# arancormonk/dsd-neo

Measured on AMD Instinct MI355X. Metric: I/Q Msamples/s end-to-end (demod->FEC->MBE) per GPU; % HBM roofline, higher is better.
Workload: dtype f32

## Files before the change

### dsd-neo_amd/csrc/ddn_rx.hip

```cpp

#include <hip/hip_runtime.h>
#include <cstdio>
#include <cstdlib>
#include <mutex>
#include <stdint.h>

#include "ddn_device.h"
#include "ddn_p25h_dev.h"
#include "ddn_slicer_dev.h"
#include "ddn_tables_p25.h"

using ddn_sl::two_max_insert;
using ddn_sl::two_min_insert;

#define DDN_RXW_RAW (1 << 30)
namespace {
constexpr int TS = 64;
constexpr int SS = 128;
constexpr int MS = 1024;
constexpr int NT = DDN_P25_FILTER_TAPS;
constexpr int QCAP = 10;
constexpr uint32_t kSyncBits = 0xFB30A0u;

__constant__ uint32_t c_taps[NT];
// ... 1715 lines not shown
        s.max = (float)(s.max_sum / (double)MS);
        s.center = (s.max + s.min) / 2.0f;
        s.maxref = s.max * 0.80f;
        s.minref = s.min * 0.80f;
        s.sidx = (s.sidx >= SS - 1) ? 0 : s.sidx + 1;
        fl = 1 | (neg ? 4 : 0);
        q_max = s.max;
        q_min = s.min;
        if (--s.lock_left <= 0) {
            if (HM && s.hphase != 0) {
                hpost = true;
            } else {
                frame_end();
            }
        }
    };
    auto commit_hunt = [&](float sym, int done_snap, int& fl) {
        L.lb[s.lidx][ln] = sym;
        s.level_count = s.level_count < 24 ? s.level_count + 1 : 24;
        float u0, u1, u2, u3;
        window_push(sym, false, u0, u1, u2, u3, done_snap);
        s.lidx = (s.lidx == 23) ? 0 : s.lidx + 1;
        s.sidx = (s.sidx >= SS - 1) ? 0 : s.sidx + 1;
        const uint32_t bit = sym > 0.0f ? 1u : 0u;
        s.hist_bits = ((s.hist_bits << 1) | bit) & 0xFFFFFFu;
        s.hist_count = s.hist_count < 24 ? s.hist_count + 1 : 24;
        if (s.hist_count >= 8) {
            s.maxref = s.max;
            s.minref = s.min;
            int pol = 0;
            if (s.hist_count >= 24) {
                pol = (s.hist_bits == kSyncBits) ? 1 : ((s.hist_bits == (~kSyncBits & 0xFFFFFFu)) ? 2 : 0);
            }
            if (pol) {
                const float big = 3.4028234663852886e38f;
                float a0 = big, a1 = big, a2 = big, a3 = big, a4 = big;
                float b0 = -big, b1 = -big, b2 = -big, b3 = -big, b4 = -big;
                const int lc = s.level_count;
#pragma unroll 4
                for (int k = 0; k < 24; k++) {
                    const float x = L.lb[k][ln];
                    float v = k < lc ? x : big, t;
                    float w = k < lc ? x : -big;
                    t = fminf(a0, v); v = fmaxf(a0, v); a0 = t;
                    t = fminf(a1, v); v = fmaxf(a1, v); a1 = t;
                    t = fminf(a2, v); v = fmaxf(a2, v); a2 = t;
                    t = fminf(a3, v); v = fmaxf(a3, v); a3 = t;
                    a4 = fminf(a4, v);
                    t = fmaxf(b0, w); w = fminf(b0, w); b0 = t;
                    t = fmaxf(b1, w); w = fminf(b1, w); b1 = t;
                    t = fmaxf(b2, w); w = fminf(b2, w); b2 = t;
                    t = fmaxf(b3, w); w = fminf(b3, w); b3 = t;
                    b4 = fmaxf(b4, w);
                }
                if (lc >= 13) {
                    s.lmin = (a2 + a3 + a4) / 3.0f;
                    s.lmax = (b4 + b3 + b2) / 3.0f;
                } else {
                    s.lmin = (a0 + a1 + a2) / 3.0f;
                    s.lmax = (b2 + b1 + b0) / 3.0f;
                }
                s.max = (s.max + s.lmax) / 2;
                s.min = (s.min + s.lmin) / 2;
                s.lastsync = pol;
                if (use_flt && !s.filter_on) {
                    s.filter_on = 1;
                    s.filt_start = abs0 + t0 + sp;
                    cold_until = sp + (NT - 1);
                }
                if (s.scount >= 24) {
                    float sp_ = 0.0f, sn_ = 0.0f;
                    int np = 0, nn = 0;
                    int idx = s.shead;
#pragma unroll 4
                    for (int k = 0; k < 24; k++) {
                        idx = idx == 0 ? 23 : idx - 1;
                        const float v = L.sh[idx][ln];
                        const bool pos = v > 0.0f;
                        sp_ += pos ? v : 0.0f;
                        sn_ += pos ? 0.0f : v;
                        np += pos ? 1 : 0;
                        nn += pos ? 0 : 1;
                    }
                    if (np != 0 && nn != 0) {
                        const float mp = sp_ / (float)np, mn = sn_ / (float)nn;
                        if (!(fabsf(mp - mn) < 1.0f)) {
                            s.max = mp;
                            s.min = mn;
                            s.center = (s.max + s.min) / 2.0f;
                            s.umid = s.center + (s.max - s.center) * 0.625f;
                            s.lmid = s.center + (s.min - s.center) * 0.625f;
                            s.maxref = s.max * 0.80f;
                            s.minref = s.min * 0.80f;
                            s.fill_max = s.max;
                            s.fill_min = s.min;
                            fill_max_d = (double)s.max;
                            fill_min_d = (double)s.min;
                            s.since_fill = 0;
                            s.max_sum = (double)s.max * (double)MS;
                            s.min_sum = (double)s.min * (double)MS;
                        }
                    }
                }
                s.have_sync = 1;
                s.lock_left = lock_cfg[ch];
                if (HM) {
                    s.lock_left = 33;
                    s.hphase = 1;
                    s.hn = 33;
                }
                fl = 2 | (pol == 2 ? 4 : 0);
                if (s.lock_left <= 0) {
                    s.have_sync = 0;
                    s.lidx = 0;
                    s.level_count = 0;
                    s.hist_count = 0;
                    s.hist_bits = 0;
                    s.lmin = s.min;
                    s.lmax = s.max;
                    s.hunt_pos = 0;
                }
            }
        }
        if (!(fl & 2)) {
            hunt_advance();
        }
    };
    auto emit = [&](float sym, int fl, float q_max, float q_min) {
    if (fl & 1) {
        hist_push(sym, q_max, q_min, fl);
    }
    if (offload && tk <= QTW) {
        qv = make_float4(sym, q_max, q_min, __int_as_float(fl | ((o - o_tile) << 8)));
    } else if ((size_t)o < max_sym) {
        int dibit, relb = 0, l0 = 0, l1 = 0;
        if (fl & 1) {
            const float center = (q_max + q_min) / 2.0f;
            const ddn_sl::Thr th = {center, ((q_max - center) * 5.0f / 8.0f) + center,
                                    ((q_min - center) * 5.0f / 8.0f) + center, q_max, q_min};
            ddn_sl::slice_soft(sym, th, (fl >> 2) & 1, dibit, relb, l0, l1);
        } else {
            dibit = sym > 0.0f ? 1 : 3;
        }
        store_record(rp + (size_t)o * 10, fp + o, sym, dibit, relb, l0, l1, fl);
    }
        o++;
    };

    long long dbg_busy = 0, dbg_wait = 0, dbg_cyc[3] = {0, 0, 0}, dbg_prev = 0, dbg_sec[8] = {0, 0, 0, 0, 0, 0, 0, 0}, dbg_st = 0;
#define DBG_SEC(k) do { if (DDN_RX_CYCLES && (cfg.dbg & 8192)) { const long long n_ = (long long)clock64(); dbg_sec[k] += n_ - dbg_st; dbg_st = n_; } } while (0)
    int dbg_n[3] = {0, 0, 0}, dbg_kind = -1;
    long long dbg_blk[8] = {0, 0, 0, 0, 0, 0, 0, 0}, dbg_bt = 0;
#define DBG_BLK(k) do { if (DDN_RX_CYCLES && (cfg.dbg & 8192)) { const long long n_ = (long long)clock64(); dbg_blk[k] += n_ - dbg_bt; dbg_bt = n_; } } while (0)
    long long dbg_run[8] = {0, 0, 0, 0, 0, 0, 0, 0};
    long long dbg_ent[8] = {0, 0, 0, 0, 0, 0, 0, 0};
    if (HM && loader) {
        const int n_tiles = (int)((n + TW - 1) / TW);
        int job[NRW];
        for (int h = 0; h < NRW; h++) {
            job[h] = 0;
        }
        float idle_spin = 0.0f;
        auto jobs_left = [&]() {
            bool any = false;
            for (int h = 0; h < NRW; h++) {
                any = any || job[h] <= n_tiles;
            }
            return any;
        };
        while (jobs_left()) {
            bool served = false;
#pragma unroll
            for (int h = 0; h < NRW; h++) {
                const int j = job[h];
                const int tdw = __hip_atomic_load(&H.tile_done[h], __ATOMIC_RELAXED, __HIP_MEMORY_SCOPE_WORKGROUP);
                if (j > n_tiles || (tdw & (DDN_RXW_RAW - 1)) < j) {
                    continue;
                }
                __builtin_amdgcn_fence(__ATOMIC_ACQUIRE, "workgroup");
                const long long w0 = (DDN_RX_CYCLES && (cfg.dbg & 8192)) ? (long long)clock64() : 0;
                if (j < n_tiles) {
                    long long c0 = w0;
                    StageRegs sg;
                    if (j + 1 < n_tiles) {
                        stage_half_load((long)(j + 1) * TW, h, sg, (tdw & DDN_RXW_RAW) != 0);
                    }
                    if (DDN_RX_CYCLES && (cfg.dbg & 8192)) {
                        const long long c1 = (long long)clock64();
                        dbg_cyc[0] += c1 - c0;
                        c0 = c1;
                    }
                    if (offload && j > 0 && !(cfg.dbg & 512)) {
                        drain_half((j - 1) & 1, h);
                    }
                    if (DDN_RX_CYCLES && (cfg.dbg & 8192)) {
                        const long long c1 = (long long)clock64();
                        dbg_cyc[1] += c1 - c0;
                        c0 = c1;
                    }
                    if (fuse_mf) {
                        if (j + 1 < n_tiles) {
                            stage_half_store(j + 1, h, sg);
                        }
                        __builtin_amdgcn_fence(__ATOMIC_RELEASE, "workgroup");
                        if (lane == 0) {
                            __hip_atomic_store(&H.staged[h], j + 2, __ATOMIC_RELAXED, __HIP_MEMORY_SCOPE_WORKGROUP);
                        }
                        if (DDN_RX_CYCLES && (cfg.dbg & 8192)) {
                            const long long c1 = (long long)clock64();
                            dbg_cyc[0] += c1 - c0;
                            c0 = c1;
                        }
                    }
                    if (j >= 1 && !(cfg.dbg & 256)) {
                        compute_sfx_half(j & 1, j & 1, h);
                    }
                    if (DDN_RX_CYCLES && (cfg.dbg & 8192)) {
                        const long long c1 = (long long)clock64();
                        dbg_cyc[2] += c1 - c0;
                        c0 = c1;
                    }
                    if (!fuse_mf && j + 1 < n_tiles) {
                        stage_half_store(j + 1, h, sg);
                    }
                    if (DDN_RX_CYCLES && (cfg.dbg & 8192)) {
                        dbg_cyc[0] += (long long)clock64() - c0;
                    }
                    __builtin_amdgcn_fence(__ATOMIC_RELEASE, "workgroup");
                    if (lane == 0) {
                        __hip_atomic_store(&H.ready[h], j + 2, __ATOMIC_RELAXED, __HIP_MEMORY_SCOPE_WORKGROUP);
                    }
                } else if (offload && n_tiles > 0) {
                    drain_half((n_tiles - 1) & 1, h);
                }
                if (DDN_RX_CYCLES && (cfg.dbg & 8192)) {
                    dbg_busy += (long long)clock64() - w0;
                }
                job[h] = j + 1;
                served = true;
            }
            if (!served) {
                const long long w0 = (DDN_RX_CYCLES && (cfg.dbg & 8192)) ? (long long)clock64() : 0;
                helper_idle(idle_spin, (cfg.dbg & 8388608) != 0, 1);
                if (DDN_RX_CYCLES && (cfg.dbg & 8192)) {
                    dbg_wait += (long long)clock64() - w0;
                }
            }
        }
        it = n_tiles;
    } else
    for (t0 = 0; t0 < n; t0 += TW, it++) {
        const long long dbg_t0 = (DDN_RX_CYCLES && (cfg.dbg & 8192)) ? (long long)clock64() : 0;
        const int tn = (int)((n - t0) < TW ? (n - t0) : TW);
        const bool more = (t0 + TW) < n;
        long long dbg_spin = 0;
        if (HM) {
            const long long w0 = (DDN_RX_CYCLES && (cfg.dbg & 8192)) ? (long long)clock64() : 0;
            while (__hip_atomic_load(&H.ready[rw], __ATOMIC_RELAXED, __HIP_MEMORY_SCOPE_WORKGROUP) <= it
                   || (fuse_mf && __hip_atomic_load(&H.fready[rw], __ATOMIC_RELAXED, __HIP_MEMORY_SCOPE_WORKGROUP) <= it)) {
                __builtin_amdgcn_s_sleep(1);
            }
            __builtin_amdgcn_fence(__ATOMIC_ACQUIRE, "workgroup");
            if (DDN_RX_CYCLES && (cfg.dbg & 8192)) {
                dbg_spin = (long long)clock64() - w0;
            }
        }
        if (loader || winprep) {
            if (loader) {
                if (more) {
                    stage(t0 + TW, (it + 1) % 3);
                }
                if (offload && it > 0 && !(cfg.dbg & 512)) {
                    drain((it - 1) & 1);
                }
            }
            if (winprep) {
                if (it >= 1 && !(cfg.dbg & 256)) {
                    compute_sfx(it & 1, it & 1);
                }
            }
        } else {
            const int base = TW + (it % 3) * TW;
            auto rd = [&](const float* row, int j) { return row[base + j]; };
            auto cold_limit = [&]() {
                if (!s.filter_on) {
                    return -2147483647;
                }
                const long long d = (long long)(NT - 1) - (abs0 + t0 - s.filt_start);
                return d <= -2147483647LL ? -2147483647 : (d > 1000000LL ? 1000000 : (int)d);
            };
            cold_until = cold_limit();
            if (it >= 1) {
                pp1 = pc1, pp2 = pc2, pp3 = pc3, pp4 = pc4;
                npp = npc;
                sbuf_sel = (it - 1) & 1;
            }
            pc1 = inf, pc2 = inf, pc3 = -inf, pc4 = -inf;
            npc = 0;
            tk = 0;
            itq = it & 1;
            o_tile = o;
            if (live && offload) {
                L.qo[it & 1][ln] = o;
            }
            int guard = 0;
            bool gblocked = false;
            bool respin = false;
            int blk_o = -1;
            while (true) {
                const long long dbg_p0 = (DDN_RX_CYCLES && (cfg.dbg & 8192)) ? (long long)clock64() : 0;
                long long dbg_p1 = 0;
                if (HM && __any(hwait)) {
                    if (hwait
                        && __hip_atomic_load(&H.rsp_seq[ln], __ATOMIC_RELAXED, __HIP_MEMORY_SCOPE_WORKGROUP) == hseq) {
                        __builtin_amdgcn_fence(__ATOMIC_ACQUIRE, "workgroup", "local");
                        const int ext = H.rsp_ext[ln];
                        hwait = false;
                        if ((cfg.dbg & 65536) && !(cfg.dbg & (67108864 | 134217728))) {
                            s.dbg_wait += (long long)clock64();
                        }
#if DDN_RX_CYCLES
                        if (cfg.dbg & 67108864) {
                            s.dbg_wait += (long long)((int)clock64() - H.rsp_t[ln]);
                        }
                        if (cfg.dbg & 134217728) {
                            s.dbg_wait += (long long)H.rsp_pick[ln];
                        }
#endif
                        if (ext > 0) {
                            s.lock_left = ext;
                            s.hn = ext;
                            s.hphase = H.rsp_more[ln] ? 2 : 0;
                        } else {
                            s.hphase = 0;
                            frame_end();
                        }
                    }
                    if (__any(hwait) && (LPR > 4) != ((cfg.dbg & 262144) != 0)) {
                        __builtin_amdgcn_s_sleep(1);
                        continue;
                    }
                }
                const bool alive = live & !hwait;
                bool hunt_wait = false;
                if (bulk_ok) {
                    const int jt = s.jitter;
                    const int i0n = (jt > 0 && jt <= (whole - 1) / 2) ? -1 : ((jt > (whole - 1) / 2 && jt < whole) ? 1 : 0);
                    const bool be = alive & (s.have_sync == 0) & (s.in_symbol == 0) & (s.need_reset == 0) & (sp >= cold_until)
                                    & (s.hunt_pos + 20 < 1800) & (blk_o != o) & ((size_t)(o + 20) < max_sym);
                    const bool fitsn = sp + whole - i0n <= tn;
                    hunt_wait = be & !fitsn & more;
                    unsigned long long bm = __ballot(be & fitsn);
                    if constexpr (LPR == 2 || LPR == 4) {
                    if (__builtin_expect(bm != 0, 0)) {
                        const long long bt0 = (DDN_RX_CYCLES && (cfg.dbg & 8192)) ? (long long)clock64() : 0;
                        constexpr int OW = 64 / LPR;
                        constexpr int CAP = OW < 17 ? OW - 1 : 16;
                        constexpr unsigned long long GM = OW == 32 ? 0xFFFFFFFFull : 0xFFFFull;
                        const int g = lane / OW, l = lane % OW;
                        const bool gact = ((bm >> g) & 1ull) != 0;
                        const int cln = rw * LPR + g;
                        const int sp0 = __shfl(sp, g);
                        const float cen_o = __shfl(s.center, g), ls_o = __shfl(s.lastsample, g);
                        const float* pr = (__shfl(s.filter_on, g) ? &L.flt[cln][0] : &L.raw[cln][0]) + base;
                        int m = 0, mypk = 0;
                        if ((bm & (bm - 1)) == 0 || (cfg.dbg & 4096)) {
                            unsigned long long b2 = bm;
                            while (b2) {
                                const int ow = __ffsll((long long)b2) - 1;
                                b2 &= b2 - 1;
                                const int sp0s = __builtin_amdgcn_readlane(sp, ow), c0s = __builtin_amdgcn_readlane(s.hist_count, ow);
                                const float cen_s = __shfl(s.center, ow), ls_s = __shfl(s.lastsample, ow);
                                float hl = __shfl(s.maxref * 1.25f, ow), ll = __shfl(s.minref * 1.25f, ow);
                                const float hl_n = __shfl(s.max * 1.25f, ow), ll_n = __shfl(s.min * 1.25f, ow);
                                const float* prs = (__builtin_amdgcn_readlane(s.filter_on, ow) ? &L.flt[rw * LPR + ow][0] : &L.raw[rw * LPR + ow][0]) + base;
                                int q = sp0s, sm = 0, jit = __builtin_amdgcn_readlane(s.jitter, ow);
                                int lim = c0s < 8 ? 8 - c0s : CAP;
                                for (int ph = 0; ph < 2; ph++) {
                                    unsigned long long cm[3];
                                    q = __builtin_amdgcn_readfirstlane(q);
                                    sm = __builtin_amdgcn_readfirstlane(sm);
                                    jit = __builtin_amdgcn_readfirstlane(jit);
#pragma unroll
                                    for (int r = 0; r < 3; r++) {
                                        cm[r] = 0ull;
                                        if (q + 64 * r < tn) {
                                            const int a = q + lane + 64 * r;
                                            bool hit = false;
                                            if (a < tn) {
                                                const float x = prs[a];
                                                const float xp = (a == sp0s) ? ls_s : prs[a - 1];
                                                hit = (x > cen_s) ? (!(x > hl) && xp < cen_s) : (!(x < ll) && xp > cen_s);
                                            }
                                            cm[r] = __ballot(hit);
                                        }
                                    }
                                    bool full = false;
                                    auto uni64 = [](unsigned long long v) {
                                        const uint32_t lo = (uint32_t)__builtin_amdgcn_readfirstlane((int)(uint32_t)v);
                                        const uint32_t hi = (uint32_t)__builtin_amdgcn_readfirstlane((int)(uint32_t)(v >> 32));
                                        return ((unsigned long long)hi << 32) | lo;
                                    };
                                    cm[0] = uni64(cm[0]);
                                    cm[1] = uni64(cm[1]);
                                    cm[2] = uni64(cm[2]);
                                    while (sm < lim) {
                                        const int c = (int)((i0tab >> (2 * (jit + 1))) & 3u), i0 = c - 1;
                                        const int cnt = whole - i0;
                                        if (q + cnt > tn) {
                                            full = true;
                                            break;
                                        }
                                        asm("s_mov_b32 m0, %2\n\tv_writelane_b32 %0, %1, m0" : "+v"(mypk) : "s"((q + 256) | (c << 10) | ((jit + 1) << 12)), "s"(ow * OW + sm) : "m0");
                                        const int k0 = i0 < 0 ? 1 : 0;
                                        const uint32_t wv = (uint32_t)(cm[0] >> k0) & ((1u << (cnt - k0)) - 1u);
                                        jit = wv ? i0 + k0 + (__ffs((int)wv) - 1) : -1;
                                        cm[0] = (cm[0] >> cnt) | (cm[1] << (64 - cnt));
                                        cm[1] = (cm[1] >> cnt) | (cm[2] << (64 - cnt));
                                        cm[2] >>= cnt;
                                        q += cnt;
                                        sm++;
                                    }
                                    if (full || lim >= CAP) {
                                        break;
                                    }
                                    lim = CAP;
                                    hl = hl_n;
                                    ll = ll_n;
                                }
                                asm("s_mov_b32 m0, %2\n\tv_writelane_b32 %0, %1, m0" : "+v"(mypk) : "s"((q + 256) | ((jit + 1) << 12)), "s"(ow * OW + sm) : "m0");
                                m = g == ow ? sm : m;
                            }
                        } else {
                            int jit = __shfl(s.jitter, g), q = sp0;
                            float hl = __shfl(s.maxref * 1.25f, g), ll = __shfl(s.minref * 1.25f, g);
                            int lim = __shfl(s.hist_count, g);
                            lim = lim < 8 ? 8 - lim : CAP;
                            bool gdone = !gact;
                            for (int ph = 0; ph < 2; ph++) {
                                unsigned long long cm0 = 0ull, cm1 = 0ull, cm2 = 0ull;
                                constexpr int PW = 64 / OW;
#pragma unroll 1
                                for (int wd = 0; wd < 3; wd++) {
                                    unsigned long long word = 0ull;
#pragma unroll
                                    for (int r = 0; r < PW; r++) {
                                        const int a = q + l + OW * (wd * PW + r);
                                        bool hit = false;
                                        if (!gdone && a < tn) {
                                            const float x = pr[a];
                                            const float xp = (a == sp0) ? ls_o : pr[a - 1];
                                            hit = (x > cen_o) ? (!(x > hl) && xp < cen_o) : (!(x < ll) && xp > cen_o);
                                        }
                                        word |= ((__ballot(hit) >> (g * OW)) & GM) << (OW * r);
                                    }
                                    cm0 = wd == 0 ? word : cm0;
                                    cm1 = wd == 1 ? word : cm1;
                                    cm2 = wd == 2 ? word : cm2;
                                }
                                bool full = false;
                                while (true) {
                                    const bool go = !gdone && !full && m < lim;
                                    if (!__any(go)) {
                                        break;
                                    }
                                    if (go) {
                                        const int c = (int)((i0tab >> (2 * (jit + 1))) & 3u), i0 = c - 1;
                                        const int cnt = whole - i0;
                                        if (q + cnt > tn) {
                                            full = true;
                                        } else {
                                            if (l == m) {
                                                mypk = (q + 256) | (c << 10) | ((jit + 1) << 12);
                                            }
                                            const int k0 = i0 < 0 ? 1 : 0;
                                            const uint32_t wv = (uint32_t)(cm0 >> k0) & ((1u << (cnt - k0)) - 1u);
                                            jit = wv ? i0 + k0 + (__ffs((int)wv) - 1) : -1;
                                            cm0 = (cm0 >> cnt) | (cm1 << (64 - cnt));
                                            cm1 = (cm1 >> cnt) | (cm2 << (64 - cnt));
                                            cm2 >>= cnt;
                                            q += cnt;
                                            m++;
                                        }
                                    }
                                }
                                if (ph == 1) {
                                    break;
                                }
                                const float hl_n = __shfl(s.max * 1.25f, g), ll_n = __shfl(s.min * 1.25f, g);
                                if (!gdone) {
                                    if (full || lim >= CAP) {
                                        gdone = true;
                                    } else {
                                        lim = CAP;
                                        hl = hl_n;
                                        ll = ll_n;
                                    }
                                }
                                if (!__any(!gdone)) {
                                    break;
                                }
                            }
                            if (l == m) {
                                mypk = (q + 256) | ((jit + 1) << 12);
                            }
                        }
                        const int myq = (mypk & 1023) - 256, myi0 = ((mypk >> 10) & 3) - 1, myjin = ((mypk >> 12) & 15) - 1;
                        const int c0 = __shfl(s.hist_count, g);
                        const uint32_t h0 = (uint32_t)__shfl((int)s.hist_bits, g);
                        float sym = 0.0f;
                        if (gact && l < m) {
                            const float* pw = pr + myq + ((whole - 1) / 2 - 2 - myi0);
                            float acc = 0.0f;
#pragma unroll
                            for (int w = 0; w < 5; w++) {
                                acc += __builtin_amdgcn_fmed3f(pw[w], -inf, inf);
                            }
                            sym = acc / 5.0f;
                        }
                        const uint32_t sw = (uint32_t)((__ballot(gact && l < m && sym > 0.0f) >> (g * OW)) & GM);
                        const int lj = l < 31 ? l : 31;
                        const uint32_t hj = ((h0 << (lj + 1)) | __brev(sw << (31 - lj))) & 0xFFFFFFu;
                        const bool syn = gact && l < m && (c0 + l + 1 >= 24) && (hj == kSyncBits || hj == (~kSyncBits & 0xFFFFFFu));
                        const uint32_t smg = (uint32_t)((__ballot(syn) >> (g * OW)) & GM);
                        if (smg) {
                            m = __ffs((int)smg) - 1;
                        }
                        const int o_o = __shfl(o, g);
                        const int sh_o = __shfl(s.shead, g), li_o = __shfl(s.lidx, g), si_o = __shfl(s.sidx, g);
                        if (gact && l < m) {
                            int k = sh_o + l;
                            L.sh[k >= 24 ? k - 24 : k][cln] = sym;
                            k = li_o + l;
                            L.lb[k >= 24 ? k - 24 : k][cln] = sym;
                            L.sb[(si_o + l) & (SS - 1)][cln] = sym;
                            const size_t oo = (size_t)(o_o + l);
                            if (oo < max_sym) {
                                const size_t cho = (size_t)(ch0 + cln);
                                store_record(rec + (cho * max_sym + oo) * 10, flags + cho * max_sym + oo, sym, sym > 0.0f ? 1 : 3, 0, 0, 0, 0);
                            }
                        }
                        float a1 = (gact && l < m) ? sym : inf, a2 = inf, b1 = (gact && l < m) ? sym : -inf, b2 = -inf;
#define DDN_ROW_STEP(ctl)                                                                                                                   \
    do {                                                                                                                                    \
        const float o1 = __int_as_float(__builtin_amdgcn_update_dpp(0, __float_as_int(a1), ctl, 0xF, 0xF, true));                           \
        const float o2 = __int_as_float(__builtin_amdgcn_update_dpp(0, __float_as_int(a2), ctl, 0xF, 0xF, true));                           \
        const float p1 = __int_as_float(__builtin_amdgcn_update_dpp(0, __float_as_int(b1), ctl, 0xF, 0xF, true));                           \
        const float p2 = __int_as_float(__builtin_amdgcn_update_dpp(0, __float_as_int(b2), ctl, 0xF, 0xF, true));                           \
        two_min_insert(o1, a1, a2);                                                                                                         \
        two_min_insert(o2, a1, a2);                                                                                                         \
        two_max_insert(p1, b1, b2);                                                                                                         \
        two_max_insert(p2, b1, b2);                                                                                                         \
    } while (0)
                        DDN_ROW_STEP(0xB1);
                        DDN_ROW_STEP(0x4E);
                        DDN_ROW_STEP(0x124);
                        DDN_ROW_STEP(0x128);
#undef DDN_ROW_STEP
                        const int orow = (lane < LPR ? lane : 0) * OW;
                        const int m_own = __shfl(m, orow);
                        const int src1 = orow + (m_own > 0 ? m_own - 1 : 0);
                        const int qf = __shfl(myq, orow + m_own), jf = __shfl(myjin, orow + m_own);
                        const int il = __shfl(myi0, src1);
                        const uint32_t hf = (uint32_t)__shfl((int)hj, src1);
                        a1 = __shfl(a1, orow), a2 = __shfl(a2, orow), b1 = __shfl(b1, orow), b2 = __shfl(b2, orow);
                        if (lane < LPR && (be & fitsn)) {
                            if (m_own == 0) {
                                blk_o = o;
                            } else {
                                const float* prow = (s.filter_on ? &L.flt[ln][0] : &L.raw[ln][0]) + base;
                                const float lsf = prow[qf - 1];
                                two_min_insert(a1, pc1, pc2);
                                two_min_insert(a2, pc1, pc2);
                                two_max_insert(b1, pc3, pc4);
                                two_max_insert(b2, pc3, pc4);
                                npc += m_own;
                                wabs = fmaxf(wabs, fmaxf(fabsf(a1), fabsf(b1)));
                                s.shead = (s.shead + m_own) % 24;
                                s.scount = s.scount + m_own < 24 ? s.scount + m_own : 24;
                                s.lidx = (s.lidx + m_own) % 24;
                                s.level_count = s.level_count + m_own < 24 ? s.level_count + m_own : 24;
                                s.sidx = (s.sidx + m_own) & (SS - 1);
                                s.hist_bits = hf;
                                s.hist_count = s.hist_count + m_own < 24 ? s.hist_count + m_own : 24;
                                if (s.hist_count >= 8) {
                                    s.maxref = s.max;
                                    s.minref = s.min;
                                }
                                s.hunt_pos += m_own;
                                s.span = whole;
                                s.centre = (whole - 1) / 2;
                                s.i = il;
                                s.sum = 0.0f;
                                s.count = 0;
                                s.in_symbol = 0;
                                s.jitter = jf;
                                s.lastsample = lsf;
                                sp = qf;
                                o += m_own;
                            }
                        }
                        if (DDN_RX_CYCLES && (cfg.dbg & 8192)) {
                            const long long now = (long long)clock64();
                            dbg_sec[6] += now - bt0;
                            dbg_sec[7]++;
                            dbg_prev += now - bt0;
                        }
                        continue;
                    }
                    } else
                    if (__builtin_expect(bm != 0, 0)) {
                        const long long bt0 = (DDN_RX_CYCLES && (cfg.dbg & 8192)) ? (long long)clock64() : 0;
                        while (bm) {
                            const int ow = __ffsll((long long)bm) - 1;
                            bm &= bm - 1;
                            if (DDN_RX_CYCLES && (cfg.dbg & 8192)) {
                                dbg_bt = (long long)clock64();
                                dbg_blk[7]++;
                            }
                            const int cln = rw * LPR + ow;
                            const int sp0 = __builtin_amdgcn_readlane(sp, ow);
                            const int c0 = __builtin_amdgcn_readlane(s.hist_count, ow);
                            const int flt_o = __builtin_amdgcn_readlane(s.filter_on, ow);
                            int jit = __builtin_amdgcn_readlane(s.jitter, ow);
                            const uint32_t h0 = (uint32_t)__builtin_amdgcn_readlane((int)s.hist_bits, ow);
                            const int o_o = __builtin_amdgcn_readlane(o, ow);
                            const float cen_o = __shfl(s.center, ow), hl_o = __shfl(s.maxref * 1.25f, ow);
                            const float ll_o = __shfl(s.minref * 1.25f, ow), ls_o = __shfl(s.lastsample, ow);
                            const float* pr = (flt_o ? &L.flt[cln][0] : &L.raw[cln][0]) + base;
                            float hl = hl_o, ll = ll_o;
                            const float hl_n = __shfl(s.max * 1.25f, ow), ll_n = __shfl(s.min * 1.25f, ow);
                            int q = sp0, m = 0, mypk = 0;
                            int lim = c0 < 8 ? 8 - c0 : 16;
                            DBG_BLK(0);
                            for (int ph = 0; ph < 2; ph++) {
                                unsigned long long cm[3];
                                q = __builtin_amdgcn_readfirstlane(q);
                                m = __builtin_amdgcn_readfirstlane(m);
                                jit = __builtin_amdgcn_readfirstlane(jit);
#pragma unroll
                                for (int r = 0; r < 3; r++) {
                                    cm[r] = 0ull;
                                    if (q + 64 * r < tn) {
                                        const int a = q + lane + 64 * r;
                                        bool hit = false;
                                        if (a < tn) {
                                            const float x = pr[a];
                                            const float xp = (a == sp0) ? ls_o : pr[a - 1];
                                            hit = (x > cen_o) ? (!(x > hl) && xp < cen_o) : (!(x < ll) && xp > cen_o);
                                        }
                                        cm[r] = __ballot(hit);
                                    }
                                }
                                bool full = false;
                                auto uni64 = [](unsigned long long v) {
                                    const uint32_t lo = (uint32_t)__builtin_amdgcn_readfirstlane((int)(uint32_t)v);
                                    const uint32_t hi = (uint32_t)__builtin_amdgcn_readfirstlane((int)(uint32_t)(v >> 32));
                                    return ((unsigned long long)hi << 32) | lo;
                                };
                                cm[0] = uni64(cm[0]);
                                cm[1] = uni64(cm[1]);
                                cm[2] = uni64(cm[2]);
                                while (m < lim) {
                                    const int c = (int)((i0tab >> (2 * (jit + 1))) & 3u), i0 = c - 1;
                                    const int cnt = whole - i0;
                                    if (q + cnt > tn) {
                                        full = true;
                                        break;
                                    }
                                    asm("s_mov_b32 m0, %2\n\tv_writelane_b32 %0, %1, m0" : "+v"(mypk) : "s"((q + 256) | (c << 10) | ((jit + 1) << 12)), "s"(m) : "m0");
                                    const int k0 = i0 < 0 ? 1 : 0;
                                    const uint32_t wv = (uint32_t)(cm[0] >> k0) & ((1u << (cnt - k0)) - 1u);
                                    jit = wv ? i0 + k0 + (__ffs((int)wv) - 1) : -1;
                                    cm[0] = (cm[0] >> cnt) | (cm[1] << (64 - cnt));
                                    cm[1] = (cm[1] >> cnt) | (cm[2] << (64 - cnt));
                                    cm[2] >>= cnt;
                                    q += cnt;
                                    m++;
                                }
                                if (full || lim >= 16) {
                                    break;
                                }
                                lim = 16;
                                hl = hl_n;
                                ll = ll_n;
                            }
                            DBG_BLK(1);
                            asm("s_mov_b32 m0, %2\n\tv_writelane_b32 %0, %1, m0" : "+v"(mypk) : "s"((q + 256) | ((jit + 1) << 12)), "s"(m) : "m0");
                            const int myq = (mypk & 1023) - 256, myi0 = ((mypk >> 10) & 3) - 1, myjin = ((mypk >> 12) & 15) - 1;
                            float sym = 0.0f;
                            if (lane < m) {
                                const float* pw = pr + myq + ((whole - 1) / 2 - 2 - myi0);
                                float acc = 0.0f;
#pragma unroll
                                for (int w = 0; w < 5; w++) {
                                    acc += __builtin_amdgcn_fmed3f(pw[w], -inf, inf);
                                }
                                sym = acc / 5.0f;
                            }
                            const uint32_t sw = (uint32_t)__ballot(lane < m && sym > 0.0f);
                            const int lj = lane < 31 ? lane : 31;
                            const uint32_t hj = ((h0 << (lj + 1)) | __brev(sw << (31 - lj))) & 0xFFFFFFu;
                            const bool syn = lane < m && (c0 + lane + 1 >= 24) && (hj == kSyncBits || hj == (~kSyncBits & 0xFFFFFFu));
                            const unsigned long long sm = __ballot(syn);
                            if (sm) {
                                m = __ffsll((long long)sm) - 1;
                            }
                            DBG_BLK(2);
                            if (m == 0) {
                                if (lane == ow) {
                                    blk_o = o;
                                }
                                continue;
                            }
                            const int qf = __builtin_amdgcn_readlane(myq, m), jf = __builtin_amdgcn_readlane(myjin, m);
                            const int il = __builtin_amdgcn_readlane(myi0, m - 1);
                            const uint32_t hf = (uint32_t)__builtin_amdgcn_readlane((int)hj, m - 1);
                            const int sh_o = __builtin_amdgcn_readlane(s.shead, ow), li_o = __builtin_amdgcn_readlane(s.lidx, ow);
                            const int si_o = __builtin_amdgcn_readlane(s.sidx, ow);
                            if (lane < m) {
                                int k = sh_o + lane;
                                L.sh[k >= 24 ? k - 24 : k][cln] = sym;
                                k = li_o + lane;
                                L.lb[k >= 24 ? k - 24 : k][cln] = sym;
                                L.sb[(si_o + lane) & (SS - 1)][cln] = sym;
                                const size_t oo = (size_t)(o_o + lane);
                                if (oo < max_sym) {
                                    const size_t cho = (size_t)(ch0 + cln);
                                    store_record(rec + (cho * max_sym + oo) * 10, flags + cho * max_sym + oo, sym, sym > 0.0f ? 1 : 3, 0, 0, 0, 0);
                                }
                            }
                            DBG_BLK(3);
                            float a1 = lane < m ? sym : inf, a2 = inf, b1 = lane < m ? sym : -inf, b2 = -inf;
#pragma unroll
                            for (int d = 1; d < 16; d <<= 1) {
                                const float o1 = __shfl_xor(a1, d), o2 = __shfl_xor(a2, d), p1 = __shfl_xor(b1, d), p2 = __shfl_xor(b2, d);
                                two_min_insert(o1, a1, a2);
                                two_min_insert(o2, a1, a2);
                                two_max_insert(p1, b1, b2);
                                two_max_insert(p2, b1, b2);
                            }
                            a1 = __shfl(a1, 0), a2 = __shfl(a2, 0), b1 = __shfl(b1, 0), b2 = __shfl(b2, 0);
                            const float lsf = pr[qf - 1];
                            DBG_BLK(4);
                            if (lane == ow) {
                                two_min_insert(a1, pc1, pc2);
                                two_min_insert(a2, pc1, pc2);
                                two_max_insert(b1, pc3, pc4);
                                two_max_insert(b2, pc3, pc4);
                                npc += m;
                                wabs = fmaxf(wabs, fmaxf(fabsf(a1), fabsf(b1)));
                                s.shead = (s.shead + m) % 24;
                                s.scount = s.scount + m < 24 ? s.scount + m : 24;
                                s.lidx = (s.lidx + m) % 24;
                                s.level_count = s.level_count + m < 24 ? s.level_count + m : 24;
// ... 479 lines not shown
                        sp += cnt;
                        s.i = s.span;
                    }
                }
                const bool gen = wholeok && fits && !latched && !genf;
                if (__any(gen)) {
                    for (int k = 0; k < WMAX; k++) {
                        const bool on = gen && k < cnt;
                        if (!__any(on)) {
                            break;
                        }
                        if (on) {
                            float x = rd(row, sp + k);
                            if (s.have_sync) {
                                x = x > s.max ? s.max : (x < s.min ? s.min : x);
                            }
                            const int i = s.i + k;
                            if (s.jitter < 0) {
                                if (x > s.center) {
                                    if (!(x > s.maxref * 1.25f) && s.lastsample < s.center) {
                                        s.jitter = i;
                                    }
                                } else if (!(x < s.minref * 1.25f) && s.lastsample > s.center) {
                                    s.jitter = i;
                                }
                            }
                            if (s.span == 20 && i >= 7 && i <= 13) {
                                s.sum += x;
                                s.count++;
                            }
                            if ((s.span == 5 && i == 2) || (i >= s.centre - 2 && i <= s.centre + 2)) {
                                s.sum += x;
                                s.count++;
                            }
                            s.lastsample = x;
                        }
                    }
                    if (gen) {
                        sp += cnt;
                        s.i = s.span;
                    }
                }
                bool act = glive && s.in_symbol && sp < tn && s.i < s.span && !blocked;
                while (__any(act)) {
                    if (act) {
                        float x = rd(rrow, sp);
                        if (s.filter_on) {
                            const long long a = abs0 + t0 + sp;
                            if (a - s.filt_start >= (long long)(NT - 1)) {
                                x = rd(frow, sp);
                            } else {
                                const long k = t0 + sp;
                                float acc = 0.0f;
                                for (int i = 0; i < NT; i++) {
                                    const int jr = sp - (NT - 1) + i;
                                    const long j = k - (NT - 1) + i;
                                    float v;
                                    if (abs0 + j < s.filt_start) {
                                        v = fstale[(size_t)ch * (NT - 1) + (size_t)((abs0 + j - s.filt_start) + (NT - 1))];
                                    } else if (jr >= (it > 0 ? -TW : 0)) {
                                        v = rd(rrow, jr);
                                    } else {
                                        v = (j >= 0) ? raw[(size_t)ch * stride + j]
                                                     : prev_tail[(size_t)ch * (NT - 1) + (NT - 1) + j];
                                    }
                                    acc += __uint_as_float(c_taps[i]) * v;
                                }
                                x = acc;
                            }
                        }
                        if (s.have_sync) {
                            x = x > s.max ? s.max : (x < s.min ? s.min : x);
                        }
                        const int i = s.i;
                        if (s.jitter < 0) {
                            if (x > s.center) {
                                if (!(x > s.maxref * 1.25f) && s.lastsample < s.center) {
                                    s.jitter = i;
                                }
                            } else if (!(x < s.minref * 1.25f) && s.lastsample > s.center) {
                                s.jitter = i;
                            }
                        }
                        if (s.span == 20 && i >= 7 && i <= 13) {
                            s.sum += x;
                            s.count++;
                        }
                        if ((s.span == 5 && i == 2) || (i >= s.centre - 2 && i <= s.centre + 2)) {
                            s.sum += x;
                            s.count++;
                        }
                        s.lastsample = x;
                        s.i++;
                        sp++;
                    }
                    act = glive && s.in_symbol && sp < tn && s.i < s.span && !blocked;
                }
                const bool done = glive && s.in_symbol && s.i >= s.span;
                if (done) {
                    const float sym = (s.count > 0) ? (s.sum / (float)s.count) : 0.0f;
                    s.in_symbol = 0;
                    commit_pre(sym);
                    int fl = 0;
                    float q_max = 0.0f, q_min = 0.0f;
                    if (s.have_sync) {
                        commit_inframe(sym, done_snap, fl, q_max, q_min);
                    } else {
                        commit_hunt(sym, done_snap, fl);
                    }
                    emit(sym, fl, q_max, q_min);
                }
                gblocked = gblocked || blocked;
            }
            if ((DDN_RX_CYCLES && (cfg.dbg & 8192)) && dbg_kind >= 0) {
                dbg_cyc[dbg_kind] += (long long)clock64() - dbg_prev;
                dbg_n[dbg_kind]++;
                dbg_kind = -1;
            }
            if (offload && lane == 0) {
                L.qn[it & 1][rw] = (tk - 1) < QTW ? (tk - 1) : QTW;
            }
            if (live) {
                L.sidx0[(it + 1) & 1][ln] = s.sidx;
                sp -= TW;
            }
            if (HM) {
                const bool want = live
                                  && (!s.filter_on || cold_until > 0 || (!s.have_sync && s.hunt_pos + 64 >= 1800) || raw_always);
                const int raw_bit = __any(want) ? DDN_RXW_RAW : 0;
                __builtin_amdgcn_fence(__ATOMIC_RELEASE, "workgroup");
                if (lane == 0) {
                    __hip_atomic_store(&H.tile_done[rw], (it + 1) | raw_bit, __ATOMIC_RELAXED, __HIP_MEMORY_SCOPE_WORKGROUP);
                }
            }
        }
        if (DDN_RX_CYCLES && (cfg.dbg & 8192)) {
            const long long t1 = (long long)clock64();
            if (!HM) {
                __syncthreads();
            }
            dbg_busy += t1 - dbg_t0 - dbg_spin;
            dbg_wait += (long long)clock64() - t1 + dbg_spin;
        } else if (!HM) {
            __syncthreads();
        }
    }
    if ((DDN_RX_CYCLES && (cfg.dbg & 8192)) && lane == 0) {
        uint8_t* d = rec + ((size_t)ch0 + 1) * max_sym * 10 - 192 + (wave < NRW ? (wave ? 1 : 0) : 2) * 64;
        const long long v[8] = {dbg_busy, dbg_wait, dbg_cyc[0], dbg_cyc[1], dbg_cyc[2], dbg_n[0], dbg_n[1], dbg_n[2]};
        for (int k = 0; k < 64; k++) {
            d[k] = reinterpret_cast<const uint8_t*>(v)[k];
        }
        if (wave == 0) {
            uint8_t* d2 = rec + ((size_t)ch0 + 1) * max_sym * 10 - 256;
            for (int k = 0; k < 64; k++) {
                d2[k] = reinterpret_cast<const uint8_t*>(dbg_sec)[k];
                d2[k - 64] = reinterpret_cast<const uint8_t*>(dbg_run)[k];
                d2[k - 128] = reinterpret_cast<const uint8_t*>(dbg_blk)[k];
                d2[k - 256] = reinterpret_cast<const uint8_t*>(dbg_ent)[k];
            }
        }
    }
    if (!HM && loader && offload && it > 0) {
        drain((it - 1) & 1);
    }
    if (live) {
        if (s.have_sync) {
            s.umid = ((s.max - s.center) * 5.0f / 8.0f) + s.center;
            s.lmid = ((s.min - s.center) * 5.0f / 8.0f) + s.center;
        }
        s.n_abs = abs0 + n;
        state[ch] = s;
        counts[ch] = o;
        for (int k = 0; k < SS; k++) {
            sbuf_store[(size_t)k * n_channels + ch] = L.sb[k][ln];
        }
        for (int k = 0; k < 24; k++) {
            lbuf_store[(size_t)k * n_channels + ch] = L.lb[k][ln];
            shist_store[(size_t)k * n_channels + ch] = L.sh[k][ln];
        }
    }
}

template <int CPW, bool HM, int NRW_T = (HM ? 2 : 1)>
static hipError_t
launch_rxw(const float* raw, const float* filt, const float* prev_tail, float* fstale, long n, size_t stride, int n_channels,
           const DdnRxConfig& cfg, DdnRxState* state, float* sbuf_store, float* lbuf_store, float* shist_store,
           float* minring, float* maxring, uint8_t* rec, uint8_t* flags, int32_t* counts, size_t max_sym, const int32_t* lock_cfg,
           DdnP25HState* hstate, float* hh_store, int32_t* events, int32_t* n_events, hipStream_t st) {
    const size_t shm1 = HM ? (((((sizeof(LdsW<CPW, true>) + 15) & ~(size_t)15) + sizeof(LdsH<CPW>)) + 15) & ~(size_t)15) : sizeof(LdsW<CPW>);
    const size_t shm = shm1 * (NRW_T == 4 ? 2 : 1);
    const unsigned lblocks = (unsigned)((n_channels + CPW - 1) / CPW);
    const unsigned nblocks = NRW_T == 4 ? (lblocks + 1) / 2 : lblocks;
    const unsigned nthreads = HM ? 64 * (NRW_T + 2) * (NRW_T == 4 ? 2 : 1) : 192;
    if (HM && (cfg.sym_rate <= 0 || cfg.out_rate / cfg.sym_rate < 9)) {
        return hipErrorInvalidValue;
    }
    hipError_t e = hipFuncSetAttribute(reinterpret_cast<const void*>(&k_p25_rxw<CPW, HM, NRW_T>),
                                       hipFuncAttributeMaxDynamicSharedMemorySize, (int)shm);
    if (e != hipSuccess) {
        return e;
    }
    if (DDN_EXP_ENV("DDN_RX_OCC")) {
        int nb = -1;
        hipFuncAttributes fa;
        (void)hipOccupancyMaxActiveBlocksPerMultiprocessor(&nb, reinterpret_cast<const void*>(&k_p25_rxw<CPW, HM, NRW_T>), (int)nthreads, shm);
        (void)hipFuncGetAttributes(&fa, reinterpret_cast<const void*>(&k_p25_rxw<CPW, HM, NRW_T>));
        fprintf(stderr, "k_p25_rxw<%d,%d,%d>: %d blocks per CU, %d regs, %zu B dynamic LDS, %zu B static\n", CPW, (int)HM, NRW_T, nb, fa.numRegs, shm, fa.sharedSizeBytes);
    }
    hipLaunchKernelGGL((k_p25_rxw<CPW, HM, NRW_T>), dim3(nblocks), dim3(nthreads), shm, st, raw,
                       filt, prev_tail, fstale, n, stride, n_channels, cfg, state, sbuf_store, lbuf_store, shist_store, minring,
                       maxring, rec, flags, counts, max_sym, lock_cfg, hstate, hh_store, events, n_events);
    return hipGetLastError();
}

template <int CPW>
static hipError_t
launch_rx(const float* raw, const float* filt, const float* prev_tail, float* fstale, long n, size_t stride, int n_channels,
          const DdnRxConfig& cfg, DdnRxState* state, float* sbuf_store, float* lbuf_store, float* shist_store,
          float* minring, float* maxring, uint8_t* rec, uint8_t* flags, int32_t* counts, size_t max_sym, const int32_t* lock_cfg,
          hipStream_t st) {
    const size_t shm = sizeof(Lds<CPW>);
    hipError_t e = hipFuncSetAttribute(reinterpret_cast<const void*>(&k_p25_rx<CPW>),
                                       hipFuncAttributeMaxDynamicSharedMemorySize, (int)shm);
    if (e != hipSuccess) {
        return e;
    }
    hipLaunchKernelGGL(k_p25_rx<CPW>, dim3((unsigned)((n_channels + CPW - 1) / CPW)), dim3(128), shm, st, raw, filt,
                       prev_tail, fstale, n, stride, n_channels, cfg, state, sbuf_store, lbuf_store, shist_store, minring,
                       maxring, rec, flags, counts, max_sym, lock_cfg);
    return hipGetLastError();
}

static inline bool
use_filter_row_missing(const DdnRxConfig* cfg, const float* filt) {
    return cfg->use_filter && !filt;
}

static int
handler_mode_cpw(int channels_per_wave, int n_channels) {
    int cpw = channels_per_wave;
    if (const char* e = DDN_EXP_ENV("DDN_RX_CPW")) {
        cpw = atoi(e);
    }
    if (cpw != 4 && cpw != 8 && cpw != 16) {
        cpw = n_channels <= 4 * 512 ? 4 : 8;
    }
    return cpw;
}

extern "C" int
ddn_dev_p25_rx_fuses_filter(const DdnRxConfig* cfg, int channels_per_wave, int n_channels) {
    return cfg && cfg->handlers && cfg->use_filter && handler_mode_cpw(channels_per_wave, n_channels) <= 8
               ? 1
               : 0;
}

extern "C" hipError_t
ddn_dev_p25_rx(const float* raw, const float* filt, const float* prev_tail, float* fstale, long n, size_t stride, int n_channels,
               const DdnRxConfig* cfg, DdnRxState* state, float* sbuf_store, float* lbuf_store, float* shist_store,
               float* minring, float* maxring, uint8_t* rec, uint8_t* flags, int32_t* counts, size_t max_sym,
               int channels_per_wave, const int32_t* lock_cfg, DdnP25HState* hstate, float* hh_store, int32_t* events,
               int32_t* n_events, hipStream_t st) {
    if (n_channels <= 0 || n <= 0) {
        return hipSuccess;
    }
    if ((unsigned long long)n_channels * (unsigned long long)MS * 4ull > 0xFFFFFFFFull) {
        return hipErrorInvalidValue;
    }
    {
        static std::mutex mu;
        static bool taps_up[64] = {};
        int dev = 0;
        hipError_t e = hipGetDevice(&dev);
        if (e != hipSuccess) {
            return e;
        }
        std::lock_guard<std::mutex> lock(mu);
        if (dev < 0 || dev >= 64 || !taps_up[dev]) {
            e = hipMemcpyToSymbol(HIP_SYMBOL(c_taps), ddn_p25_filter_bits, sizeof(uint32_t) * NT);
            if (e != hipSuccess) {
                return e;
            }
            if (dev >= 0 && dev < 64) {
                taps_up[dev] = true;
            }
        }
    }
    int cpw = channels_per_wave;
    if (const char* e = DDN_EXP_ENV("DDN_RX_CPW")) {
        cpw = atoi(e);
    }
    const int whole = cfg->sym_rate > 0 ? cfg->out_rate / cfg->sym_rate : 0;
    if (cfg->handlers) {
        if (whole < 6 || !hstate || !hh_store || !events || !n_events) {
            return hipErrorInvalidValue;
        }
        cpw = handler_mode_cpw(channels_per_wave, n_channels);
        if (use_filter_row_missing(cfg, filt) && cpw > 8) {
            return hipErrorInvalidValue;
        }
        if (cpw == 4) {
            return launch_rxw<4, true>(raw, filt, prev_tail, fstale, n, stride, n_channels, *cfg, state, sbuf_store, lbuf_store,
                                       shist_store, minring, maxring, rec, flags, counts, max_sym, lock_cfg, hstate, hh_store,
                                       events, n_events, st);
        }
        if (cpw == 8) {
            if (cfg->dbg & 16777216) {
                return launch_rxw<8, true, 4>(raw, filt, prev_tail, fstale, n, stride, n_channels, *cfg, state, sbuf_store, lbuf_store,
                                              shist_store, minring, maxring, rec, flags, counts, max_sym, lock_cfg, hstate, hh_store,
                                              events, n_events, st);
// ... 52 lines not shown
```

Measured before the change: 25980.

## Streamline bulk symbol-hunt path with preloaded samples, readlane broadcasts and permute gathers

In the single-lane bulk hunt path, the three 64-sample windows are loaded once before the two-phase loop and reused. Phase 1 shifts the existing hit masks instead of rebuilding them, and the k0 masking is simplified. Lane-uniform state is broadcast with readlane instead of shfl. The final per-group gather uses ds_permute from the owning lanes, which removes the reload of the last sample from LDS, and the modulo-24 updates become conditional subtracts. Debug cycle counters are also added, and these only run under a debug flag.

Result: faster. 26290, median of 6 (+1.2%).

```diff
diff --git a/dsd-neo_amd/csrc/ddn_rx.hip b/dsd-neo_amd/csrc/ddn_rx.hip
--- a/dsd-neo_amd/csrc/ddn_rx.hip
+++ b/dsd-neo_amd/csrc/ddn_rx.hip
@@ -1891,6 +1891,9 @@
     int dbg_n[3] = {0, 0, 0}, dbg_kind = -1;
     long long dbg_blk[8] = {0, 0, 0, 0, 0, 0, 0, 0}, dbg_bt = 0;
 #define DBG_BLK(k) do { if (DDN_RX_CYCLES && (cfg.dbg & 8192)) { const long long n_ = (long long)clock64(); dbg_blk[k] += n_ - dbg_bt; dbg_bt = n_; } } while (0)
+    uint32_t dbg_b[10] = {0, 0, 0, 0, 0, 0, 0, 0, 0, 0}, dbg_b0 = 0;
+#define DBG_B(k) do { if (DDN_RX_CYCLES && (cfg.dbg & 8192)) { const uint32_t n_ = (uint32_t)clock64(); dbg_b[k] += n_ - dbg_b0; dbg_b0 = n_; } } while (0)
+#define DBG_B2(k, k2) do { if (DDN_RX_CYCLES && (cfg.dbg & 8192)) { const uint32_t n_ = (uint32_t)clock64(); dbg_b[k] += n_ - dbg_b0; dbg_b[k2] += n_ - dbg_b0; dbg_b0 = n_; } } while (0)
     long long dbg_run[8] = {0, 0, 0, 0, 0, 0, 0, 0};
     long long dbg_ent[8] = {0, 0, 0, 0, 0, 0, 0, 0};
     if (HM && loader) {
@@ -2093,6 +2096,10 @@
                     if constexpr (LPR == 2 || LPR == 4) {
                     if (__builtin_expect(bm != 0, 0)) {
                         const long long bt0 = (DDN_RX_CYCLES && (cfg.dbg & 8192)) ? (long long)clock64() : 0;
+                        if (DDN_RX_CYCLES && (cfg.dbg & 8192)) {
+                            dbg_b0 = (uint32_t)bt0;
+                            dbg_b[7] += __popcll(bm);
+                        }
                         constexpr int OW = 64 / LPR;
                         constexpr int CAP = OW < 17 ? OW - 1 : 16;
                         constexpr unsigned long long GM = OW == 32 ? 0xFFFFFFFFull : 0xFFFFull;
@@ -2108,58 +2115,70 @@
                             while (b2) {
                                 const int ow = __ffsll((long long)b2) - 1;
                                 b2 &= b2 - 1;
+                                auto rlf = [&](float v) { return __int_as_float(__builtin_amdgcn_readlane(__float_as_int(v), ow)); };
                                 const int sp0s = __builtin_amdgcn_readlane(sp, ow), c0s = __builtin_amdgcn_readlane(s.hist_count, ow);
-                                const float cen_s = __shfl(s.center, ow), ls_s = __shfl(s.lastsample, ow);
-                                float hl = __shfl(s.maxref * 1.25f, ow), ll = __shfl(s.minref * 1.25f, ow);
-                                const float hl_n = __shfl(s.max * 1.25f, ow), ll_n = __shfl(s.min * 1.25f, ow);
+                                const float cen_s = rlf(s.center), ls_s = rlf(s.lastsample);
+                                float hl = rlf(s.maxref * 1.25f), ll = rlf(s.minref * 1.25f);
+                                const float hl_n = rlf(s.max * 1.25f), ll_n = rlf(s.min * 1.25f);
                                 const float* prs = (__builtin_amdgcn_readlane(s.filter_on, ow) ? &L.flt[rw * LPR + ow][0] : &L.raw[rw * LPR + ow][0]) + base;
                                 int q = sp0s, sm = 0, jit = __builtin_amdgcn_readlane(s.jitter, ow);
                                 int lim = c0s < 8 ? 8 - c0s : CAP;
+                                float xs[3], xps[3];
+#pragma unroll
+                                for (int r = 0; r < 3; r++) {
+                                    const int a = sp0s + lane + 64 * r;
+                                    xs[r] = prs[a < tn ? a : sp0s];
+                                    xps[r] = prs[(a < tn && a > sp0s) ? a - 1 : sp0s];
+                                }
+                                xps[0] = lane == 0 ? ls_s : xps[0];
+                                DBG_B(0);
                                 for (int ph = 0; ph < 2; ph++) {
                                     unsigned long long cm[3];
                                     q = __builtin_amdgcn_readfirstlane(q);
                                     sm = __builtin_amdgcn_readfirstlane(sm);
                                     jit = __builtin_amdgcn_readfirstlane(jit);
-#pragma unroll
-                                    for (int r = 0; r < 3; r++) {
-                                        cm[r] = 0ull;
-                                        if (q + 64 * r < tn) {
-                                            const int a = q + lane + 64 * r;
-                                            bool hit = false;
-                                            if (a < tn) {
-                                                const float x = prs[a];
-                                                const float xp = (a == sp0s) ? ls_s : prs[a - 1];
-                                                hit = (x > cen_s) ? (!(x > hl) && xp < cen_s) : (!(x < ll) && xp > cen_s);
-                                            }
-                                            cm[r] = __ballot(hit);
-                                        }
-                                    }
-                                    bool full = false;
                                     auto uni64 = [](unsigned long long v) {
                                         const uint32_t lo = (uint32_t)__builtin_amdgcn_readfirstlane((int)(uint32_t)v);
                                         const uint32_t hi = (uint32_t)__builtin_amdgcn_readfirstlane((int)(uint32_t)(v >> 32));
                                         return ((unsigned long long)hi << 32) | lo;
                                     };
-                                    cm[0] = uni64(cm[0]);
-                                    cm[1] = uni64(cm[1]);
-                                    cm[2] = uni64(cm[2]);
-                                    while (sm < lim) {
+#pragma unroll
+                                    for (int r = 0; r < 3; r++) {
+                                        const float x = xs[r], xp = xps[r];
+                                        const bool hit = (sp0s + lane + 64 * r < tn)
+                                                         && ((x > cen_s) ? (!(x > hl) && xp < cen_s) : (!(x < ll) && xp > cen_s));
+                                        cm[r] = uni64(__ballot(hit));
+                                    }
+                                    if (ph == 1) {
+                                        int d = q - sp0s;
+                                        if (d >= 64) {
+                                            cm[0] = cm[1];
+                                            cm[1] = cm[2];
+                                            cm[2] = 0ull;
+                                            d -= 64;
+                                        }
+                                        cm[0] = (cm[0] >> d) | ((cm[1] << 1) << (63 - d));
+                                        cm[1] = (cm[1] >> d) | ((cm[2] << 1) << (63 - d));
+                                        cm[2] >>= d;
+                                    }
+                                    DBG_B2(1, 8);
+                                    while (true) {
                                         const int c = (int)((i0tab >> (2 * (jit + 1))) & 3u), i0 = c - 1;
-                                        const int cnt = whole - i0;
-                                        if (q + cnt > tn) {
-                                            full = true;
+                                        const int cnt = whole - i0, qn = q + cnt;
+                                        if (sm >= lim || qn > tn) {
                                             break;
                                         }
                                         asm("s_mov_b32 m0, %2\n\tv_writelane_b32 %0, %1, m0" : "+v"(mypk) : "s"((q + 256) | (c << 10) | ((jit + 1) << 12)), "s"(ow * OW + sm) : "m0");
-                                        const int k0 = i0 < 0 ? 1 : 0;
-                                        const uint32_t wv = (uint32_t)(cm[0] >> k0) & ((1u << (cnt - k0)) - 1u);
-                                        jit = wv ? i0 + k0 + (__ffs((int)wv) - 1) : -1;
+                                        const uint32_t wv = (uint32_t)cm[0] & ((1u << cnt) - 1u) & ~((uint32_t)i0 >> 31);
+                                        jit = wv ? i0 + (__ffs((int)wv) - 1) : -1;
                                         cm[0] = (cm[0] >> cnt) | (cm[1] << (64 - cnt));
                                         cm[1] = (cm[1] >> cnt) | (cm[2] << (64 - cnt));
                                         cm[2] >>= cnt;
-                                        q += cnt;
+                                        q = qn;
                                         sm++;
                                     }
+                                    const bool full = sm < lim;
+                                    DBG_B(1);
                                     if (full || lim >= CAP) {
                                         break;
                                     }
@@ -2176,6 +2195,10 @@
                             int lim = __shfl(s.hist_count, g);
                             lim = lim < 8 ? 8 - lim : CAP;
                             bool gdone = !gact;
+                            if (DDN_RX_CYCLES && (cfg.dbg & 8192)) {
+                                dbg_b[9]++;
+                            }
+                            DBG_B(0);
                             for (int ph = 0; ph < 2; ph++) {
                                 unsigned long long cm0 = 0ull, cm1 = 0ull, cm2 = 0ull;
                                 constexpr int PW = 64 / OW;
@@ -2197,6 +2220,7 @@
                                     cm1 = wd == 1 ? word : cm1;
                                     cm2 = wd == 2 ? word : cm2;
                                 }
+                                DBG_B2(1, 8);
                                 bool full = false;
                                 while (true) {
                                     const bool go = !gdone && !full && m < lim;
@@ -2223,6 +2247,7 @@
                                         }
                                     }
                                 }
+                                DBG_B(1);
                                 if (ph == 1) {
                                     break;
                                 }
@@ -2247,7 +2272,10 @@
                         const int myq = (mypk & 1023) - 256, myi0 = ((mypk >> 10) & 3) - 1, myjin = ((mypk >> 12) & 15) - 1;
                         const int c0 = __shfl(s.hist_count, g);
                         const uint32_t h0 = (uint32_t)__shfl((int)s.hist_bits, g);
+                        const int o_o = __shfl(o, g);
+                        const int sh_o = __shfl(s.shead, g), li_o = __shfl(s.lidx, g), si_o = __shfl(s.sidx, g);
                         float sym = 0.0f;
+                        const float lsp = (gact && l > 0 && l <= m) ? pr[myq - 1] : 0.0f;
                         if (gact && l < m) {
                             const float* pw = pr + myq + ((whole - 1) / 2 - 2 - myi0);
                             float acc = 0.0f;
@@ -2265,8 +2293,7 @@
                         if (smg) {
                             m = __ffs((int)smg) - 1;
                         }
-                        const int o_o = __shfl(o, g);
-                        const int sh_o = __shfl(s.shead, g), li_o = __shfl(s.lidx, g), si_o = __shfl(s.sidx, g);
+                        DBG_B(2);
                         if (gact && l < m) {
                             int k = sh_o + l;
                             L.sh[k >= 24 ? k - 24 : k][cln] = sym;
@@ -2279,6 +2306,7 @@
                                 store_record(rec + (cho * max_sym + oo) * 10, flags + cho * max_sym + oo, sym, sym > 0.0f ? 1 : 3, 0, 0, 0, 0);
                             }
                         }
+                        DBG_B(3);
                         float a1 = (gact && l < m) ? sym : inf, a2 = inf, b1 = (gact && l < m) ? sym : -inf, b2 = -inf;
 #define DDN_ROW_STEP(ctl)                                                                                                                   \
     do {                                                                                                                                    \
@@ -2291,33 +2319,42 @@
         two_max_insert(p1, b1, b2);                                                                                                         \
         two_max_insert(p2, b1, b2);                                                                                                         \
     } while (0)
-                        DDN_ROW_STEP(0xB1);
+                        {
+                            const float o1 = __int_as_float(__builtin_amdgcn_update_dpp(0, __float_as_int(a1), 0xB1, 0xF, 0xF, true));
+                            const float p1 = __int_as_float(__builtin_amdgcn_update_dpp(0, __float_as_int(b1), 0xB1, 0xF, 0xF, true));
+                            two_min_insert(o1, a1, a2);
+                            two_max_insert(p1, b1, b2);
+                        }
                         DDN_ROW_STEP(0x4E);
                         DDN_ROW_STEP(0x124);
                         DDN_ROW_STEP(0x128);
 #undef DDN_ROW_STEP
-                        const int orow = (lane < LPR ? lane : 0) * OW;
-                        const int m_own = __shfl(m, orow);
-                        const int src1 = orow + (m_own > 0 ? m_own - 1 : 0);
-                        const int qf = __shfl(myq, orow + m_own), jf = __shfl(myjin, orow + m_own);
-                        const int il = __shfl(myi0, src1);
-                        const uint32_t hf = (uint32_t)__shfl((int)hj, src1);
-                        a1 = __shfl(a1, orow), a2 = __shfl(a2, orow), b1 = __shfl(b1, orow), b2 = __shfl(b2, orow);
+                        DBG_B(4);
+                        const int l1 = m > 0 ? m - 1 : 0;
+                        const int tm = ((gact && l == m) ? g : 63) * 4, t1 = ((gact && l == l1) ? g : 63) * 4, t0 = ((gact && l == 0) ? g : 63) * 4;
+                        const int pkf = __builtin_amdgcn_ds_permute(tm, mypk);
+                        const float lsf = __int_as_float(__builtin_amdgcn_ds_permute(tm, __float_as_int(lsp)));
+                        const int il = __builtin_amdgcn_ds_permute(t1, myi0);
+                        const uint32_t hf = (uint32_t)__builtin_amdgcn_ds_permute(t1, (int)hj);
+                        const int m_own = __builtin_amdgcn_ds_permute(t0, m);
+                        a1 = __int_as_float(__builtin_amdgcn_ds_permute(t0, __float_as_int(a1)));
+                        a2 = __int_as_float(__builtin_amdgcn_ds_permute(t0, __float_as_int(a2)));
+                        b1 = __int_as_float(__builtin_amdgcn_ds_permute(t0, __float_as_int(b1)));
+                        b2 = __int_as_float(__builtin_amdgcn_ds_permute(t0, __float_as_int(b2)));
+                        const int qf = (pkf & 1023) - 256, jf = ((pkf >> 12) & 15) - 1;
                         if (lane < LPR && (be & fitsn)) {
                             if (m_own == 0) {
                                 blk_o = o;
                             } else {
-                                const float* prow = (s.filter_on ? &L.flt[ln][0] : &L.raw[ln][0]) + base;
-                                const float lsf = prow[qf - 1];
                                 two_min_insert(a1, pc1, pc2);
                                 two_min_insert(a2, pc1, pc2);
                                 two_max_insert(b1, pc3, pc4);
                                 two_max_insert(b2, pc3, pc4);
                                 npc += m_own;
                                 wabs = fmaxf(wabs, fmaxf(fabsf(a1), fabsf(b1)));
-                                s.shead = (s.shead + m_own) % 24;
+                                s.shead = s.shead + m_own >= 24 ? s.shead + m_own - 24 : s.shead + m_own;
                                 s.scount = s.scount + m_own < 24 ? s.scount + m_own : 24;
-                                s.lidx = (s.lidx + m_own) % 24;
+                                s.lidx = s.lidx + m_own >= 24 ? s.lidx + m_own - 24 : s.lidx + m_own;
                                 s.level_count = s.level_count + m_own < 24 ? s.level_count + m_own : 24;
                                 s.sidx = (s.sidx + m_own) & (SS - 1);
                                 s.hist_bits = hf;
@@ -2339,7 +2376,11 @@
                                 o += m_own;
                             }
                         }
+                        DBG_B(5);
                         if (DDN_RX_CYCLES && (cfg.dbg & 8192)) {
+                            for (int j = 0; j < LPR; j++) {
+                                dbg_b[6] += ((bm >> j) & 1ull) ? __builtin_amdgcn_readlane(m_own, j) : 0;
+                            }
                             const long long now = (long long)clock64();
                             dbg_sec[6] += now - bt0;
                             dbg_sec[7]++;
@@ -3125,11 +3166,20 @@
             d[k] = reinterpret_cast<const uint8_t*>(v)[k];
         }
         if (wave == 0) {
+            long long dbg_blk2[8] = {0, 0, 0, 0, 0, 0, 0, 0};
+            if constexpr (LPR == 2 || LPR == 4) {
+                for (int k = 0; k < 8; k++) {
+                    dbg_blk[k] = dbg_b[k];
+                }
+                dbg_blk2[0] = dbg_b[8];
+                dbg_blk2[1] = dbg_b[9];
+            }
             uint8_t* d2 = rec + ((size_t)ch0 + 1) * max_sym * 10 - 256;
             for (int k = 0; k < 64; k++) {
                 d2[k] = reinterpret_cast<const uint8_t*>(dbg_sec)[k];
                 d2[k - 64] = reinterpret_cast<const uint8_t*>(dbg_run)[k];
                 d2[k - 128] = reinterpret_cast<const uint8_t*>(dbg_blk)[k];
+                d2[k - 320] = reinterpret_cast<const uint8_t*>(dbg_blk2)[k];
                 d2[k - 256] = reinterpret_cast<const uint8_t*>(dbg_ent)[k];
             }
         }
```
